# klkuhlm/unconfined

Measured on AMD Instinct MI355X. Metric: (t,r) drawdown points/sec, Neuman-1974 1024x256 sweep; max |rel err| vs CPU ref, higher is better.
Workload: dtype f64

## Files before the change

unconfined_amd/csrc/ucf_device.h:

```cpp

#include "ucf_math.h"
#include "ucf_plan.h"
#include <cstdlib>

namespace UCF_NS {

using namespace ucfm;

#define UCF_STR_(x) #x
#define UCF_STR(x) UCF_STR_(x)
#define UCF_PI 3.14159265358979323846
#define UCF_EPS 2.220446049250313e-16

UCF_DEV double shfl_down1(double v) { return __shfl_down(v, 1, 64); }
UCF_DEV double shift_down1(double x)
{
    const int lo = __double2loint(x), hi = __double2hiint(x);
    const int l2 = __builtin_amdgcn_update_dpp(lo, lo, 0x130, 0xf, 0xf, false);
    const int h2 = __builtin_amdgcn_update_dpp(hi, hi, 0x130, 0xf, 0xf, false);
    return __hiloint2double(h2, l2);
}
UCF_DEV cplx shfl_down1(cplx v) { return cmake(shift_down1(v.re), shift_down1(v.im)); }
UCF_DEV cplx bcast0(cplx v) { return cmake(__shfl(v.re, 0, 64), __shfl(v.im, 0, 64)); }
UCF_DEV double wave_max(double v)
{
#pragma unroll
    for (int off = 32; off >= 1; off >>= 1) v = fmax(v, __shfl_xor(v, off, 64));
    return v;
}
UCF_DEV void stat_add(long long* ctr, bool pred)
{
    if (ctr == nullptr) return;
    unsigned long long bal = __ballot(pred);
    if (bal != 0ull && (threadIdx.x & 63) == 0) atomicAdd((unsigned long long*)ctr, (unsigned long long)__popcll(bal));
}

#ifndef UCF_TU
#define UCF_TU -1
#endif
#define UCF_TU_HAS(L) (UCF_TU < 0 || UCF_TU == (L))

typedef double2 lds_c;
UCF_DEV cplx lds_ld(const lds_c* base, int slot, int lane) { lds_c v = base[slot * UCF_WAVE + lane]; return cmake(v.x, v.y); }
UCF_DEV void lds_st(lds_c* base, int slot, int lane, cplx z) { base[slot * UCF_WAVE + lane] = make_double2(z.re, z.im); }
#define UCF_PART 16
template <int PART = UCF_PART>
UCF_DEV cplx scr_ld(const lds_c* base, int slot, int lane) { lds_c v = base[slot * PART + (lane & (PART - 1))]; return cmake(v.x, v.y); }
template <int PART = UCF_PART>
UCF_DEV void scr_st(lds_c* base, int slot, int lane, cplx z) { base[slot * PART + (lane & (PART - 1))] = make_double2(z.re, z.im); }

#if UCF_FAST
UCF_DEV cplx cinv_plain_(cplx z)
{
    const double r = fast_rcp(z.re * z.re + z.im * z.im);
    return cmake(z.re * r, -(z.im * r));
}
#endif

UCF_DEV cplx lap_time(const ucf_dev_params& P, cplx p)
{
    if (P.timeType < 0) {
        const bool linear = P.timeType <= -101;
        const int n = linear ? -P.timeType - 100 : -P.timeType;
        cplx sum = cmake(0.0, 0.0);
        for (int k = 0; k < n; k++) {
            const cplx term = rscale(P.sched[n + k], cexp_(rscale(-P.sched[k], p)));
            sum = (k == 0) ? term : cadd(sum, term);
        }
        const cplx num = csub(sum, rscale(P.sched[2 * n + 1], cexp_(rscale(-P.sched[2 * n], p))));
        return cdiv(num, linear ? cmul(p, p) : p);
    }
    const double t1 = P.timePar[0], t2 = P.timePar[1];
    switch (P.timeType) {
    case 1: return cdiv(cexp_(cscale(p, -t1)), p);
    case 2: return csub(cdiv(cexp_(cscale(p, -t1)), p), cdiv(cexp_(cscale(p, -t2)), p));
    case 3: return cexp_(cscale(p, -t1));
    case 4: {
        cplx a = rdiv(1.0, csub(p, cmul(p, cexp_(cscale(p, -t1)))));
        cplx b = rsub(1.0, cexp_(cscale(p, -t2)));
        return cdiv(cmul(a, b), p);
    }
    case 5: return cdiv(cexp_(cscale(p, -t2)), cadd(p, cmul(p, cexp_(cscale(p, -t1)))));
    case 6: return cdiv(cmul(cexp_(cscale(p, -t2)), p), caddr(cmul(p, p), t1 * t1));
    case 7: return cmake(0.0, 0.0);
    case 8: {
        cplx ex = cexp_(cdivr(cscale(p, -t1), 2.0));
        cplx num = cmul(cexp_(cscale(p, -t2)), rsub(1.0, ex));
        return cdiv(num, cmul(radd(1.0, ex), p));
    }
    default: return cmake(__builtin_nan(""), __builtin_nan(""));
    }
}

struct k01 { cplx k0, k1; int ierr; };
UCF_DEV cplx clog_(cplx z) { return cmake(log(hypot(z.re, z.im)), atan2(z.im, z.re)); }

__device__ __noinline__ static k01 cbesk01_(cplx z)
{
    k01 out;
    out.k0 = cmake(0.0, 0.0); out.k1 = out.k0; out.ierr = 0;
    const double tol = UCF_EPS;
    const double elim = 2.303 * (1021.0 * log10(2.0) - 3.0);
    const double alim = elim + fmax(-(log10(2.0) * 52.0 * 2.303), -41.45);
    const double at1 = 0.78539816339744830962;
    const double pi = 4.0 * at1, hpi = 2.0 * at1, spi = 3.0 / (2.0 * at1);
    const double rthpi = sqrt(8.0 * at1) / 2.0, fpi = 1.89769999331517738, tth = 6.66666666666666666e-01;
    const double gamma_e = 5.77215664901532861e-01;
    const double xx = z.re, yy = z.im;
    if (xx == 0.0 && yy == 0.0) { out.ierr = 1; return out; }
    const double caz = hypot(xx, yy);
    if (caz > 1073741823.5) { out.ierr = 4; return out; }
    if (caz < UCF_DBL_MIN * 1.0e3) { out.ierr = 2; return out; }
    if (!(caz > tol) && -log(0.5 * caz) > elim) { out.ierr = 2; return out; }
    const cplx rz = cdiv(cmake(2.0, 0.0), z);
    cplx s1, s2;
    if (caz <= 2.0) {
        const cplx smu = clog_(rz);
        cplx f = cadd(rscale(-gamma_e, cmake(1.0, 0.0)), cscale(smu, 1.0));
        cplx p = cmake(0.5, 0.0), q = cmake(0.5, 0.0);
        s1 = f; s2 = p;
        double ak = 1.0, a1 = 1.0, bk = 1.0;
        cplx ck = cmake(1.0, 0.0);
        if (caz >= tol) {
            const cplx cz = cscale(cmul(z, z), 0.25);
            const double t1 = 0.25 * caz * caz;
            do {
                f = cdivr(cadd(cadd(cscale(f, ak), p), q), bk);
                p = cdivr(p, ak);
                q = cdivr(q, ak);
                const double rk = 1.0 / ak;
                ck = cscale(cmul(ck, cz), rk);
                s1 = cadd(s1, cmul(ck, f));
                s2 = cadd(s2, cmul(ck, csub(p, cscale(f, ak))));
                a1 = a1 * t1 * rk;
                bk = bk + ak + ak + 1.0;
                ak = ak + 1.0;
            } while (a1 > tol);
        }
        out.k0 = s1;
        out.k1 = cmul(s2, rz);
        return out;
    }
    if (xx > alim) { out.ierr = 2; return out; }
    cplx coef = cdiv(cmake(rthpi, 0.0), csqrt_(z));
    {
        double sn, cs;
        sincos_(yy, &sn, &cs);
        coef = cmul(coef, rscale(exp(-xx), cmake(cs, -sn)));
    }
    double ak = fabs(cos(pi * 0.0));
    double fhs = 0.25;
    double t1 = 52.0 * log10(2.0) * 3.321928094;
    t1 = fmin(fmax(t1, 12.0), 60.0);
    const double t2 = tth * t1 - 6.0;
    t1 = (xx == 0.0) ? hpi : fabs(atan(yy / xx));
    double fk;
// ... 1065 lines not shown
            }
        };
        for (; n < nabs; n++) {
            const double2 aa = row[n];
            sample_common S;
            S.clean3 = resume;
            sample_prepare<FAMILY>(P, aa.x, p, need_lay1, S, fdbuf, lane, lane_aux);
            for (int z = 0; z < nz; z++) {
                const cplx f = sample_z<FAMILY>(P, S, z);
                accumulate(n, aa.y, z, f);
            }
        }
        finish_item<LAYOUT, UCF_PART>(P, accTS, scr, areas_lds ? accGL : nullptr, areas, arg, W, pt, tD, tee, p, st, nt, ir0, totlap,
                                      hout, dhout);
    }
}

#if UCF_FAST
template <int FAMILY, bool MULTI>
__global__ void __launch_bounds__(256)
laptime_kernel(const ucf_dev_params P0, int nrows, const double* __restrict__ tDv, double2* __restrict__ ltab,
               const ucf_dev_params* __restrict__ Pv, int ppp, int pbase)
{
    const long long gid = (long long)blockIdx.x * blockDim.x + threadIdx.x;
    if (gid >= (long long)nrows * P0.np) return;
    const int m = (int)(gid / nrows), row = (int)(gid % nrows);
    const ucf_dev_params& P = item_params<MULTI>(P0, Pv, row + pbase, ppp);
    const double tee = 2.0 * tDv[row];
    const double sigma = P.alpha - P.logtol / (2.0 * tee);
    const cplx p = cmake(sigma, UCF_PI * m / tee);
    cplx lt = cscale(lap_time(P, p), fast_scale<FAMILY>(P));
    if (FAMILY == 5) lt = cmul(lt, cdiv(hstorage_A0(P, p), caddr(cscale(p, P.hs_tDb), 1.0)));
    ltab[gid] = make_double2(lt.re, lt.im);
}

#ifndef UCF_FOLD_WAVES
#define UCF_FOLD_WAVES 5
#endif
#ifndef UCF_UNFOLD_WAVES
#define UCF_UNFOLD_WAVES 4
#endif
#ifndef UCF_TAIL_LSPLIT_DEFAULT
#define UCF_TAIL_LSPLIT_DEFAULT 3
#endif
#ifndef UCF_KV
#define UCF_KV(FAMILY, FOLD) ((FAMILY) == 4 ? 0 : 4)
#endif
template <int FAMILY, int LAYOUT, int WAVES, bool MULTI, bool FOLD, bool LAY3, int NZC = 0, bool LAY1 = true, bool NOFOLD = false>
__global__ void __launch_bounds__(UCF_WAVE * UCF_IWPB, WAVES)
integrate_kernel(const ucf_dev_params P0, int npts, int per_point, int nr, int nsv, int svmin,
                 const double* __restrict__ tDv, const double* __restrict__ rDv, const int* __restrict__ svv,
                 const double2* __restrict__ tab, int nt, int ir0, double2* __restrict__ state, int* __restrict__ ndone,
                 int* __restrict__ todo, const ucf_dev_params* __restrict__ Pv, int ppp, int pbase, int lsplit,
                 const double2* __restrict__ ltab, int nrows, int nheadw, int nworkw, int* __restrict__ wcount)
{
    extern __shared__ lds_c lds[];
#ifdef UCF_K1_ASSUME
    const ucf_dev_params& P = P0;
    UCF_K1_ASSUME
#endif
    const int lane = threadIdx.x & (UCF_WAVE - 1), wv = __builtin_amdgcn_readfirstlane(threadIdx.x / UCF_WAVE);
    constexpr int EF = (FAMILY == 5) ? 1 : FAMILY;
    constexpr bool ZPAIR = FOLD && EF == 2 && NZC == 1;
    const int nz = NZC ? NZC : P0.nz, R = P0.R, nacc = P0.nacc, N = P0.N, ngl = P0.ngl;
    __builtin_assume(nz >= 1 && R >= 1 && nacc >= 1 && ngl >= 1);
    const int nabs = N + nacc * ngl;
    {
        const double2* __restrict__ gt = (const double2*)P0.sc_tab;
        for (int k = threadIdx.x; k < UCF_SC_ENTRIES; k += UCF_WAVE * UCF_IWPB) lds[k] = gt[k];
    }
    __syncthreads();
    const lds_c* sct = lds;
    const int lslots = (NZC ? R : R + 1) * nz;
    lds_c* const wlds = lds + UCF_SC_ENTRIES + (size_t)wv * lslots * UCF_WAVE;
    lds_c* accTS = wlds;
    lds_c* accCur = wlds + (size_t)R * nz * UCF_WAVE;
    int ustat = blockIdx.x * UCF_IWPB + wv - gridDim.x * UCF_IWPB;
    auto next_unit = [&]() {
        if (!wcount) return ustat += gridDim.x * UCF_IWPB;
        int u = 0;
        if (lane == 0) u = __hip_atomic_fetch_add(wcount, 1, __ATOMIC_RELAXED, __HIP_MEMORY_SCOPE_AGENT);
        return __builtin_amdgcn_readfirstlane(u);
    };
    for (int wi = next_unit(); wi < nworkw; wi = next_unit()) {
        const bool tail = wi >= nheadw;
        const int ls = tail ? (lsplit >> 8) : (lsplit & 255), nsplit = 1 << ls;
        const int wj = tail ? wi - nheadw : wi;
        const int pt = (tail ? (nheadw >> (lsplit & 255)) : 0) + (wj >> ls), sub = wj & (nsplit - 1);
        auto part_bound = [&](int k) {
            if (k <= 0) return 0;
            if (k >= nsplit) return nabs;
            int j = (k * nabs / nsplit - N + ngl / 2) / ngl;
            j = j < 0 ? 0 : (j > nacc ? nacc : j);
            return N + j * ngl;
        };
        const int n0 = part_bound(sub), n1 = part_bound(sub + 1);
        if (n1 <= n0 && sub != 0) continue;
#ifdef UCF_TIMELINE
        const unsigned long long tl_t0 = __builtin_amdgcn_s_memtime();
#endif
        const work_item W = decode_item<LAYOUT>(P0, pt, lane, per_point, nr, nt, ir0, npts);
        const ucf_dev_params& P = item_params<MULTI>(P0, Pv, (LAYOUT == 3 ? W.plan * ppp : W.pidx) + pbase, ppp);
        bool need_lay1 = false, need_lay3 = false, need_lay12 = false;
        for (int z = 0; z < nz; z++) { need_lay1 |= (P.zLay[z] == 1); need_lay3 |= (P.zLay[z] == 3); need_lay12 |= (P.zLay[z] != 3); }
        const double tD = tDv[W.it], rD = rDv[W.ir];
        const int sv = (LAYOUT == 1) ? svmin : svv[W.it];
        const double2* __restrict__ row = tab + (size_t)(per_point ? W.pidx : (W.ir * nsv + (sv - svmin))) * nabs;
        const double tee = 2.0 * tD;
        const double sigma = P.alpha - P.logtol / (2.0 * tee);
        const cplx p = cmake(sigma, UCF_PI * W.mlap / tee);
        const double2 ltv = ltab[(size_t)(W.mlap < P0.np ? W.mlap : P0.np - 1) * nrows + W.it];
        const cplx lt = cmake(ltv.x, ltv.y);
        const lane_consts LC = make_lane_consts(P, p, lt);
        auto lt_again = [&]() {
            int it = W.it;
            asm volatile("" : "+v"(it));
            const double2 v = ltab[(size_t)(W.mlap < P0.np ? W.mlap : P0.np - 1) * nrows + it];
            return cmake(v.x, v.y);
        };
        double2* __restrict__ sti = state + (size_t)pt * state_slots(P0) * UCF_WAVE;
        double2* __restrict__ areas = sti + (size_t)(R + 1) * nz * UCF_WAVE;
        for (int s = 0; s < lslots; s++) lds_st(wlds, s, lane, cmake(0.0, 0.0));
        fast_common F;
        sc_ctx_init(F.sc, sct, UCF_KV(FAMILY, FOLD));
        const bool lane_ok = FAMILY != 2 || (fabs(LC.xifac.re) + fabs(LC.xifac.im) < 1.0e90);
        const int nlim = (__builtin_amdgcn_ballot_w64(!lane_ok) == 0) ? n1 : n0;

        int n = n0;
        double2 aa = row[n0 < nabs ? n0 : 0];
        int m = 0, jj = n0 > N ? (n0 - N) / ngl : 0;
        cplx acc0 = cmake(0.0, 0.0), acc1 = cmake(0.0, 0.0);
        int zph = 0;
        if constexpr (ZPAIR) {
            int stopped = 0;
            zph = 0;
            if (!MULTI && nlim > n0)
                zph = zpair_part_phase(P, LC, P.j0z[sv - 1 + (nlim > N ? (nlim - N + ngl - 1) / ngl : 0)] / rD);
            const int nts = nlim < N ? nlim : N;
            for (; n < nts; n++) {
                const double2 nxt = row[n + 1 < nabs ? n + 1 : n];
                F.sc.salt = n;
                if (!fast_eta_wave_zpair<!MULTI>(P, LC, aa.x, F, zph, 1)) { stopped = 1; break; }
                const cplx val = rscale(aa.y, fast_sample_zpair<!MULTI>(P, LC, F, zph, 1));
                const int n1 = n + 1;
                int tz = __builtin_ctz(n1);
                if (tz > R - 1) tz = R - 1;
                for (int sh = 0; sh <= tz; sh++) {
                    const int j = R - sh;
                    const double wl = P.ts_w[(size_t)(j - 1) * N + ((n1 >> sh) - 1)];
                    lds_st(accTS, j - 1, lane, cadd(lds_ld(accTS, j - 1, lane), rscale(wl, val)));
                }
                aa = nxt;
            }
            if (!stopped) for (; n < nlim; n++) {
                const double2 nxt = row[n + 1 < nabs ? n + 1 : n];
                F.sc.salt = n;
                const int last = m == ngl - 1;
                if (!fast_eta_wave_zpair<!MULTI>(P, LC, aa.x, F, zph, last)) break;
                const cplx fz = fast_sample_zpair<!MULTI>(P, LC, F, zph, last);
                acc0 = cmake(__builtin_fma(fz.re, aa.y, acc0.re), __builtin_fma(fz.im, aa.y, acc0.im));
                if (++m == ngl) {
                    const double lob = P.j0z[sv + jj - 1] / rD;
                    const double hib = P.j0z[sv + jj] / rD;
                    const double hw = (hib - lob) / 2.0;
                    const cplx ar = cmul(rscale(hw, acc0), lt_again());
                    areas[(size_t)jj * UCF_WAVE + lane] = make_double2(ar.re, ar.im);
                    acc0 = cmake(0.0, 0.0);
                    m = 0;
                    jj++;
                }
                aa = nxt;
            }
        } else
        for (; n < nlim; n++) {
            const double2 nxt = row[n + 1 < nabs ? n + 1 : n];
            const bool ts = n < N;
            F.sc.salt = n;
            if (!fast_eta_wave<EF, ZPAIR>(P, LC, aa.x, F)) break;
            if constexpr (!ZPAIR) fast_common_terms<EF, FOLD, LAY3, LAY1, NOFOLD, ZPAIR>(P, LC, aa.x, need_lay1, F, need_lay3, need_lay12);
            const int n1 = n + 1;
            int tz = __builtin_ctz(n1);
            if (tz > R - 1) tz = R - 1;
            for (int z = 0; z < nz; z++) {
                cplx fz;
                if constexpr (ZPAIR) fz = fast_sample_zpair<!MULTI>(P, LC, F, zph, 0);
                else fz = fast_sample_z<EF, FOLD, LAY3, LAY1, NOFOLD, ZPAIR>(P, F, z);
                if (ts) {
                    const cplx val = rscale(aa.y, fz);
                    for (int sh = 0; sh <= tz; sh++) {
                        const int j = R - sh;
                        const double wl = P.ts_w[(size_t)(j - 1) * N + ((n1 >> sh) - 1)];
                        const int slot = (j - 1) * nz + z;
                        lds_st(accTS, slot, lane, cadd(lds_ld(accTS, slot, lane), rscale(wl, val)));
                    }
                } else if (nz == 1 || (NZC == 2 && z == 0)) {
                    acc0 = cmake(__builtin_fma(fz.re, aa.y, acc0.re), __builtin_fma(fz.im, aa.y, acc0.im));
                } else if (NZC == 2) {
                    acc1 = cmake(__builtin_fma(fz.re, aa.y, acc1.re), __builtin_fma(fz.im, aa.y, acc1.im));
                } else {
                    const cplx a1 = lds_ld(accCur, z, lane);
                    lds_st(accCur, z, lane, cmake(__builtin_fma(fz.re, aa.y, a1.re), __builtin_fma(fz.im, aa.y, a1.im)));
                }
            }
            if (!ts && ++m == ngl) {
                const double lob = P.j0z[sv + jj - 1] / rD;
                const double hib = P.j0z[sv + jj] / rD;
                const double hw = (hib - lob) / 2.0;
                for (int z = 0; z < nz; z++) {
                    const cplx run = (nz == 1 || (NZC == 2 && z == 0)) ? acc0 : (NZC == 2 ? acc1 : lds_ld(accCur, z, lane));
                    const cplx ar = cmul(rscale(hw, run), lt);
                    areas[(size_t)(jj * nz + z) * UCF_WAVE + lane] = make_double2(ar.re, ar.im);
                    if (nz != 1 && NZC != 2) lds_st(accCur, z, lane, cmake(0.0, 0.0));
                }
                acc0 = acc1 = cmake(0.0, 0.0);
                m = 0;
                jj++;
            }
            aa = nxt;
        }
        if (sub == 0) {
            const cplx lte = ZPAIR ? lt_again() : lt;
            for (int s = 0; s < R * nz; s++) {
                const cplx v = cmul(lds_ld(wlds, s, lane), lte);
                sti[(size_t)s * UCF_WAVE + lane] = make_double2(v.re, v.im);
            }
            for (int s = R * nz; s < (R + 1) * nz; s++) sti[(size_t)s * UCF_WAVE + lane] = make_double2(0.0, 0.0);
        }
#ifdef UCF_TIMELINE
        if (sub == 0) {
            const unsigned long long tl_t1 = __builtin_amdgcn_s_memtime();
            const unsigned hwid = __builtin_amdgcn_s_getreg(63492);
            if (lane == 0) sti[(size_t)(R * nz) * UCF_WAVE + 0] = make_double2(__longlong_as_double((long long)tl_t0), __longlong_as_double((long long)tl_t1));
            if (lane == 1) sti[(size_t)(R * nz) * UCF_WAVE + 1] = make_double2((double)hwid, (double)__builtin_amdgcn_s_getreg(63508));
        }
#endif
        if (n < n1 && lane == 0) {
            const int nrep = (n < N) ? n : n - m;
            if (atomicMin(&ndone[pt], nrep) == nabs) todo[1 + atomicAdd(&todo[0], 1)] = pt;
        }
    }
}

#endif

template <int FAMILY, int LAYOUT>
__global__ void __launch_bounds__(UCF_WAVE, 3)
integrate_generic_kernel(const ucf_dev_params P, int npts, int per_point, int nr, int nsv, int svmin,
                         const double* __restrict__ tDv, const double* __restrict__ rDv, const int* __restrict__ svv,
                         const double2* __restrict__ tab, int nt, int ir0, double2* __restrict__ state, int* __restrict__ ndone)
{
    extern __shared__ lds_c lds[];
    const int lane = threadIdx.x;
    const int nz = P.nz, R = P.R, nacc = P.nacc, N = P.N, ngl = P.ngl;
    const int nabs = N + nacc * ngl;
    lds_c* accTS = lds;
    lds_c* accCur = lds + (size_t)R * nz * UCF_WAVE;
    lds_c* fdbuf = accCur + (size_t)nz * UCF_WAVE;
    bool need_lay1 = false;
    for (int z = 0; z < nz; z++) need_lay1 |= (P.zLay[z] == 1);
    for (int pt = blockIdx.x; pt < npts; pt += gridDim.x) {
        const work_item W = decode_item<LAYOUT>(P, pt, lane, per_point, nr, nt, ir0, npts);
        const double tD = tDv[W.it], rD = rDv[W.ir];
        const int sv = (LAYOUT == 1) ? svmin : svv[W.it];
        const double2* __restrict__ row = tab + (size_t)(per_point ? W.pidx : (W.ir * nsv + (sv - svmin))) * nabs;
        const double tee = 2.0 * tD;
        const double sigma = P.alpha - P.logtol / (2.0 * tee);
        const cplx p = cmake(sigma, UCF_PI * W.mlap / tee);
        const cplx lt = lap_time(P, p);
        const cplx lane_aux = (FAMILY == 5) ? hstorage_A0(P, p) : cmake(0.0, 0.0);
        double2* __restrict__ sti = state + (size_t)pt * state_slots(P) * UCF_WAVE;
        double2* __restrict__ areas = sti + (size_t)(R + 1) * nz * UCF_WAVE;
        for (int s = 0; s < (R + 1) * nz; s++) lds_st(lds, s, lane, cmake(0.0, 0.0));
        int m = 0, jj = 0;
        for (int n = 0; n < nabs; n++) {
            const double2 aa = row[n];
            sample_common S;
            S.clean3 = false;
            sample_prepare<FAMILY>(P, aa.x, p, need_lay1, S, fdbuf, lane, lane_aux);
            const bool ts = n < N;
            for (int z = 0; z < nz; z++) {
                const cplx val = cmul(rscale(aa.y, sample_z<FAMILY>(P, S, z)), lt);
                if (ts) {
                    const int n1 = n + 1;
                    for (int j = 1; j <= R; j++) {
                        const int sh = R - j;
                        if ((n1 & ((1 << sh) - 1)) == 0) {
                            const double w = P.ts_w[(size_t)(j - 1) * N + ((n1 >> sh) - 1)];
                            const int slot = (j - 1) * nz + z;
                            lds_st(accTS, slot, lane, cadd(lds_ld(accTS, slot, lane), rscale(w, val)));
                        }
                    }
                } else {
                    cplx acc = cadd(lds_ld(accCur, z, lane), cscale(val, P.tab_premul ? 1.0 : P.gl_w[m]));
                    if (m == ngl - 1) {
                        const double lob = P.j0z[sv + jj - 1] / rD;
                        const double hib = P.j0z[sv + jj] / rD;
                        acc = rscale((hib - lob) / 2.0, acc);
                        areas[(size_t)(jj * nz + z) * UCF_WAVE + lane] = make_double2(acc.re, acc.im);
                        acc = cmake(0.0, 0.0);
                    }
                    lds_st(accCur, z, lane, acc);
                }
            }
            if (!ts && ++m == ngl) { m = 0; jj++; }
        }
        for (int s = 0; s < (R + 1) * nz; s++) sti[(size_t)s * UCF_WAVE + lane] = lds[s * UCF_WAVE + lane];
        if (lane == 0) ndone[pt] = nabs;
    }
}

template <int LAYOUT, int PART, bool WREG, int MODE = 0>
__global__ void __launch_bounds__(UCF_WAVE, (LAYOUT == 0 || (WREG && MODE != 1)) ? 3 : 4)
finish_kernel(const ucf_dev_params P, int npts, int per_point, int nr, int nsv, int svmin,
              const double* __restrict__ tDv, const double* __restrict__ rDv, const int* __restrict__ svv,
              double* __restrict__ hout, double* __restrict__ dhout, ucf_stats* st, int nt, int ir0,
              double2* __restrict__ totlap, const double2* __restrict__ state, const int* __restrict__ ndone, int* __restrict__ defer)
{
    extern __shared__ lds_c lds[];
    const int lane = threadIdx.x;
    const int nz = P.nz, R = P.R, nacc = P.nacc;
    const int nabs = P.N + nacc * P.ngl;
    lds_c* accTS = lds;
    lds_c* scr = lds + (size_t)R * nz * UCF_WAVE;
    const int nloop = (MODE == 2) ? defer[0] : npts;
    for (int wi = blockIdx.x; wi < nloop; wi += gridDim.x) {
// ... 831 lines not shown
```

unconfined_amd/csrc/ucf_fastpath.h:

```cpp
#pragma once

namespace UCF_NS {

#define UCF_UNIFORM_BLOCK() asm volatile("" ::: "memory")
#define UCF_UNIFORM_BLOCK_F(FAMILY) do { if constexpr ((FAMILY) != 4) UCF_UNIFORM_BLOCK(); } while (0)

struct fprim {
    double ch, sh, ei, sn, cs;
};

template <bool POS, bool SMALLY = false>
UCF_DEV fprim prim_from_e(double x, double ax, double e, double ei, double y, const sc_ctx& sc)
{
    const int salt = sc.salt;
    fprim f;
    f.ei = ei;
    const double he = 0.5 * e;
    f.ch = __builtin_fma(0.5, ei, he);
    double s;
    if (ax < 0.35) {
        const double x2 = ax * ax;
        double pl = addk(mulk(x2, UCF_KHERE(1.0 / 6227020800.0, salt)), UCF_KHERE(1.0 / 39916800.0, salt));
        pl = fmak(pl, x2, UCF_KHERE(1.0 / 362880.0, salt));
        pl = fmak(pl, x2, UCF_KHERE(1.0 / 5040.0, salt));
// ... 46 lines not shown
    f.sh = 0.5 * (e - ei);
    f.sn = __builtin_fma(a.sn, b.cs, -(a.cs * b.sn));
    f.cs = __builtin_fma(a.cs, b.cs, a.sn * b.sn);
    return f;
}
UCF_DEV cplx pcosh(const fprim& f) { return cmake(f.ch * f.cs, f.sh * f.sn); }
UCF_DEV cplx psinh(const fprim& f) { return cmake(f.sh * f.cs, f.ch * f.sn); }
UCF_DEV cplx pexpneg(const fprim& f) { return cmake(f.ei * f.cs, -(f.ei * f.sn)); }

UCF_DEV cplx expneg_direct(double x, double y, const sc_ctx& sc)
{
    const double ei = exp_tab_(-x, sc);
    double sn, cs;
    sincos_tab_(y, sc, &sn, &cs);
    return cmake(ei * cs, -(ei * sn));
}

UCF_DEV cplx expneg_small(double x, double y, const sc_ctx& sc)
{
    const double ei = exp_tab_(-x, sc);
    double sn, cs;
    sincos_small_(y, sc, &sn, &cs);
    return cmake(ei * cs, -(ei * sn));
}
UCF_DEV void prim_pair_small(double x, double y, double zD, double xcap, const sc_ctx& sc, fprim* f, fprim* fz)
{
    double xc;
    asm("v_min_f64 %0, %1, %2" : "=v"(xc) : "v"(x), "s"(xcap));
    const double xz = xc * zD;
    const double e = exp_tab_(xc, sc), ez = exp_tab_(xz, sc);
    const double r = fast_rcp(e * ez);
    *f = prim_from_e<true, true>(xc, xc, e, r * ez, y, sc);
    *fz = prim_from_e<true, true>(xz, xz, ez, r * e, y * zD, sc);
}

UCF_DEV cplx cfma(cplx a, cplx b, cplx c)
{
    return cmake(__builtin_fma(a.re, b.re, __builtin_fma(-a.im, b.im, c.re)), __builtin_fma(a.re, b.im, __builtin_fma(a.im, b.re, c.im)));
}
UCF_DEV cplx cfnma(cplx a, cplx b, cplx c)
{
    return cmake(__builtin_fma(-a.re, b.re, __builtin_fma(a.im, b.im, c.re)), __builtin_fma(-a.re, b.im, __builtin_fma(-a.im, b.re, c.im)));
}
UCF_DEV cplx cinv_plain(cplx z)
{
    const double r = fast_rcp(z.re * z.re + z.im * z.im);
    return cmake(z.re * r, -(z.im * r));
}
UCF_DEV cplx cinv_scaled(cplx z)
{
    const double m = fmax(fabs(z.re), fabs(z.im));
    const int il = __builtin_amdgcn_frexp_exp(m) - 1;
    const double c = ldexp(z.re, -il), d = ldexp(z.im, -il);
    const double r = fast_rcp(c * c + d * d);
    return cmake(ldexp(c * r, -il), ldexp(-(d * r), -il));
}

UCF_DEV cplx cinv_auto(cplx z)
{
    const double m = fmax(fabs(z.re), fabs(z.im));
    if (__builtin_amdgcn_ballot_w64(!(m < 1.0e150 && m > 1.0e-150)) == 0) return cinv_plain(z);
    return cinv_scaled(z);
}

struct lane_consts {
    cplx p, lt, xifac;
    cplx fdB1;
    cplx mnpv;
};

UCF_DEV lane_consts make_lane_consts(const ucf_dev_params& P, cplx p, cplx lt)
{
    lane_consts L;
    L.p = p;
    L.lt = lt;
    cplx xf = rscale(P.alphaD, cinv_plain(p));
    if (P.model == 3) {
        cplx sum = cmake(0.0, 0.0);
        for (int j = 0; j < P.MoenchM; j++) sum = cadd(sum, cinv_plain(radd(1.0, cscale(p, P.MoenchInvGamma[j]))));
        xf = cmul(cscale(xf, (double)P.MoenchM), cinv_plain(sum));
    }
    L.xifac = xf;
    L.fdB1 = cscale(cscale(cscale(p, P.fd_beta0), P.fd_expmb2), P.inv_kappa);
    L.mnpv = radd(1.0, cscale(p, P.mn_vartheta * P.mn_c3));
    return L;
}

struct fast_common {
    sc_ctx sc;
    cplx th, eta, ff1, ff2, inv_she, she, che, top, g3, inv_den, ex1;
    cplx chz0;
    fprim p1;
    int have_p1;
    cplx mn_uod;
#ifdef UCF_SINGLE_RCP
    cplx q, den;
#endif
    cplx fd_s1;
    cplx top3, fd_s13;
    bool small_eta, fd_use, fd_use3;
    int any_small, any_large;
};

template <int FAMILY>
UCF_DEV double fast_scale(const ucf_dev_params& P)
{
    if (FAMILY == 0 || FAMILY == 3) return 2.0;
    if (FAMILY == 5) return P.inv_bD;
    return (FAMILY == 2 && P.model == 4) ? 2.0 : 2.0 * P.inv_bD;
}

template <int FAMILY, bool PAIR = false>
UCF_DEV bool fast_eta(const ucf_dev_params& P, const lane_consts& L, double a, fast_common& S)
{
    const double a2 = a * a;
    const cplx q = caddr(L.p, a2);
#ifdef UCF_SINGLE_RCP
    S.q = q;
#endif
    double mq = 0.0;
    if (PAIR && FAMILY != 0) {
        double r;
        rsq_pair(q.re * q.re + q.im * q.im, &mq, &r);
        S.th = cmake(q.re * r, -(q.im * r));
    } else {
        const double r = fast_rcp(q.re * q.re + q.im * q.im);
        S.th = cmake(q.re * r, -(q.im * r));
    }
    if (FAMILY == 0) return q.re > 0.0;
    {
        const double qr = q.re * P.inv_kappa, qi = q.im * P.inv_kappa;
        double r, hr;
        const double d = PAIR ? mq * P.inv_kappa : sqrt_only(__builtin_fma(qr, qr, qi * qi));
        sqrt_hrsqrt(0.5 * (d + qr), &r, &hr);
        S.eta = cmake(r, qi * hr);
    }
    return (S.eta.re <= P.fast_eta_max) & (q.re > 0.0) & (fabs(S.eta.im) < P.fast_im_max);
}
template <int FAMILY, bool PAIR = false>
UCF_DEV bool fast_eta_wave(const ucf_dev_params& P, const lane_consts& L, double a, fast_common& S)
{
    (void)fast_eta<FAMILY, PAIR>(P, L, a, S);
    const cplx q = caddr(L.p, a * a);
    unsigned long long bad = __builtin_amdgcn_ballot_w64(!(q.re > 0.0));
    if (FAMILY != 0) {
        bad |= __builtin_amdgcn_ballot_w64(!(S.eta.re <= P.fast_eta_max));
        bad |= __builtin_amdgcn_ballot_w64(!(fabs(S.eta.im) < P.fast_im_max));
    }
    return bad == 0;
}

#ifndef UCF_ZPAIR_PHASES
#define UCF_ZPAIR_PHASES 3
#endif
enum {
    UCF_PH_RANGE = 1,
    UCF_PH_IM = 2,
    UCF_PH_LARGE = 4,
    UCF_PH_YS = 8,
    UCF_PH_YL = 16
};
UCF_DEV int zpair_part_phase(const ucf_dev_params& P, const lane_consts& L, double a_max)
{
    if (!(UCF_ZPAIR_PHASES & 2)) return 0;
    const double lim = 0.99 * P.fast_eta_max;
    const bool ok = (L.p.re > 0.0) & (lim > 0.0) & ((__builtin_fma(a_max, a_max, fabs(L.p.re) + fabs(L.p.im)) * P.inv_kappa) < lim * lim);
    return __builtin_amdgcn_ballot_w64(!ok) == 0 ? UCF_PH_RANGE : 0;
}
template <bool UNI>
UCF_DEV bool fast_eta_wave_zpair(const ucf_dev_params& P, const lane_consts& L, double a, fast_common& S, int& ph, int may_set)
{
    if constexpr (!UNI) return fast_eta_wave<2, true>(P, L, a, S);
    (void)fast_eta<2, true>(P, L, a, S);
    unsigned long long bad = 0;
    if (!(ph & UCF_PH_RANGE)) {
        const cplx q = caddr(L.p, a * a);
        bad |= __builtin_amdgcn_ballot_w64(!(q.re > 0.0));
        bad |= __builtin_amdgcn_ballot_w64(!(S.eta.re <= P.fast_eta_max));
        UCF_UNIFORM_BLOCK();
    }
    if (!(ph & UCF_PH_IM)) {
        const double ai = fabs(S.eta.im);
        bad |= __builtin_amdgcn_ballot_w64(!(ai < P.fast_im_max));
        if ((UCF_ZPAIR_PHASES & 2) && may_set && __builtin_amdgcn_ballot_w64(!(ai < 0.5 * P.fast_im_max)) == 0) ph |= UCF_PH_IM;
        UCF_UNIFORM_BLOCK();
    }
    return bad == 0;
}

template <int FAMILY, bool FOLD = false, bool LAY3 = true, bool LAY1 = true, bool NOFOLD = false, bool ZPAIR = false>
UCF_DEV void fast_common_terms(const ucf_dev_params& P, const lane_consts& L, double a, bool need_lay1_in, fast_common& S,
                               bool need_lay3_in = false, bool need_lay12 = true)
{
    static_assert(!ZPAIR || (FOLD && FAMILY == 2), "ZPAIR: folded water-table kernels only");
    const double a2 = a * a;
    if (FAMILY == 0) return;
    if (FAMILY == 3) {
        const fprim p1 = prim<true>(S.eta.re, S.eta.im, S.sc);
        S.che = pcosh(p1);
        S.she = psinh(p1);
        const double wr = __builtin_fma(a2, P.mn_c3, L.mnpv.re), wi = L.mnpv.im;
        double vr, hr;
        sqrt_hrsqrt(0.5 * (sqrt_only(__builtin_fma(wr, wr, wi * wi)) + wr), &vr, &hr);
        const cplx u = cmake(P.mn_u0 * (1.0 - vr), -(P.mn_u0 * (wi * hr)));
        const cplx Delta0 = cfnma(u, S.che, cmul(S.eta, S.she));
        S.mn_uod = cmul(u, cinv_auto(Delta0));
        return;
    }
    const bool hantush = NOFOLD || !(FAMILY == 2 && P.model == 4);
    const bool z1 = FOLD || (!NOFOLD && P.fold_dD != 0), z2 = FOLD || (!NOFOLD && P.fold_lD1 != 0);
    const bool need_lay1 = (FOLD || !LAY1) ? false : need_lay1_in;
    const bool need_lay3 = (FOLD || !LAY3) ? false : need_lay3_in;
    S.small_eta = (FAMILY != 2) || (S.eta.re < P.maxexp);
    S.any_small = ((FAMILY != 2) || (__builtin_amdgcn_ballot_w64(S.small_eta) != 0)) ? 1 : 0;
    S.any_large = ((FAMILY == 2) && (__builtin_amdgcn_ballot_w64(!S.small_eta) != 0)) ? 1 : 0;
    const bool need_p1 = (hantush && (!(z1 && z2) || need_lay1)) || FAMILY == 4 || (FAMILY == 2 && S.any_small);
    S.have_p1 = (need_p1 && !z2) ? 1 : 0;
    fprim p1;
    if (ZPAIR && need_p1) {
        fprim pz;
        prim_pair(S.eta.re, S.eta.im, P.zD[0], P.maxexp, S.sc, &p1, &pz);
        S.chz0 = pcosh(pz);
        S.che = pcosh(p1);
        S.she = psinh(p1);
        S.ex1 = cmake(0.0, 0.0);
    } else if (need_p1) {
        p1 = prim<true>(S.eta.re, S.eta.im, S.sc);
        if (!z2) S.p1 = p1;
        S.che = pcosh(p1);
        S.she = psinh(p1);
        if (need_lay1) S.ex1 = pexpneg(p1);
        else S.ex1 = cmake(0.0, 0.0);
    } else {
        S.che = S.she = S.ex1 = cmake(0.0, 0.0);
    }
    if (hantush) {
        fprim pd;
        if (!z1) { pd = prim<true>(S.eta.re * P.dD, S.eta.im * P.dD, S.sc); S.ff1 = psinh(pd); }
        else S.ff1 = cmake(0.0, 0.0);
        fprim pl;
        if (!z2) { pl = prim<true>(S.eta.re * P.lD1, S.eta.im * P.lD1, S.sc); S.ff2 = psinh(pl); }
        else S.ff2 = cmake(0.0, 0.0);
        if (!(z1 && z2) || need_lay1) S.inv_she = cinv_auto(S.she);
        if (need_lay1) {
            const cplx exl = z2 ? cmake(1.0, 0.0) : pexpneg(pl);
            S.g3 = csub(exl, cmul(cadd(S.ff1, cmul(S.ex1, S.ff2)), S.inv_she));
        }
        if (FAMILY != 1) {
            S.top = S.top3 = S.th;
            if (!(z1 && z2)) {
                if (need_lay12) {
                    cplx g1;
                    if (z1) g1 = cmake(1.0, 0.0);
                    else if (P.share_g1top == 1) g1 = pcosh(pd);
                    else if (P.share_g1top == 2) g1 = csub(pcosh(pd), cmul(rscale(P.g1_delta, S.eta), S.ff1));
                    else { const double c = P.dD1 - 1.0; g1 = pcosh(prim(S.eta.re * c, S.eta.im * c, S.sc)); }
                    const cplx udp = csub(g1, cmul(cadd(cmul(S.ff1, S.che), S.ff2), S.inv_she));
                    S.top = cmul(udp, S.th);
                }
                if (need_lay3) {
                    cplx sd1 = S.she;
                    if (!z1) {
                        const double x1 = S.eta.re * P.dD1;
                        if (__builtin_amdgcn_ballot_w64(!(x1 >= 1.0)) == 0) sd1 = psinh(prim_difference(p1, pd));
                        else sd1 = psinh(prim(x1, S.eta.im * P.dD1, S.sc));
                    }
                    const cplx udp = cmul(z2 ? sd1 : csub(sd1, S.ff2), S.inv_she);
                    S.top3 = cmul(udp, S.th);
                }
            }
        }
    } else {
        S.top = S.top3 = S.th;
    }
    if (FAMILY == 2) {
        const cplx xi = cmul(S.eta, L.xifac);
        if (P.beta != 0.0) {
            const cplx one_bex = radd(1.0, cmul(rscale(P.beta, S.eta), xi));
            if (S.small_eta) S.inv_den = cinv_plain(cfma(one_bex, S.che, cmul(xi, S.she)));
            else S.inv_den = cinv_plain(cadd(one_bex, xi));
        } else {
            if (S.small_eta) S.inv_den = cinv_plain(cfma(xi, S.she, S.che));
            else S.inv_den = cinv_plain(radd(1.0, xi));
        }
#ifdef UCF_SINGLE_RCP
        if (FOLD || !hantush) {
            cplx den;
            if (P.beta != 0.0) {
                const cplx one_bex = radd(1.0, cmul(rscale(P.beta, S.eta), xi));
                den = S.small_eta ? cfma(one_bex, S.che, cmul(xi, S.she)) : cadd(one_bex, xi);
            } else {
                den = S.small_eta ? cfma(xi, S.she, S.che) : radd(1.0, xi);
            }
            S.den = den;
            S.inv_den = cinv_auto(cmul(S.q, den));
        }
#endif
    }
    if (FAMILY == 4) {
        const int n = P.order;
        const double h = P.fd_h, invhsq = P.fd_invhsq, b3h = P.fd_beta3 / h;
        const double B2 = a2 * P.inv_kappa;
        const double csup = invhsq - b3h, K = csup * invhsq, bmid = b3h - 2.0 * invhsq - B2;
        const cplx B1 = L.fdB1;
        const cplx cc = cmake((b3h - invhsq - B2) - B1.re * P.fd_e[0], -(B1.im * P.fd_e[0]));
        const cplx eoh = cscale(S.eta, 1.0 / h);
        const cplx b1 = csub(cmul(cc, S.che), cmul(eoh, S.she));
        (void)n;
        const cplx iB2 = fd_inverse_B2(P, B1, bmid, invhsq, b3h, K);
        const cplx a2v = cscale(S.che, invhsq);
        const cplx B1p = csub(b1, cmul(rscale(csup, a2v), iB2));
        const cplx iB1p = cinv_scaled(B1p);
        const cplx v1 = cneg(cmul(cc, S.top)), v2 = rscale(-invhsq, S.top);
        const cplx v1p = csub(v1, cmul(rscale(csup, iB2), v2));
        S.fd_s1 = cmul(v1p, iB1p);
        S.fd_use = (fabs(S.fd_s1.re) + fabs(S.fd_s1.im)) > 2.3e-308;
        S.fd_s13 = S.fd_s1;
        S.fd_use3 = S.fd_use;
        if (need_lay3) {
            const cplx w1 = cneg(cmul(cc, S.top3)), w2 = rscale(-invhsq, S.top3);
            S.fd_s13 = cmul(csub(w1, cmul(rscale(csup, iB2), w2)), iB1p);
            S.fd_use3 = (fabs(S.fd_s13.re) + fabs(S.fd_s13.im)) > 2.3e-308;
        }
    }
}

template <int FAMILY>
UCF_DEV bool fast_prepare(const ucf_dev_params& P, const lane_consts& L, double a, bool need_lay1, fast_common& S)
{
    if (!fast_eta<FAMILY>(P, L, a, S)) return false;
    bool need_lay3 = false, need_lay12 = false;
    for (int z = 0; z < P.nz; z++) { need_lay3 |= (P.zLay[z] == 3); need_lay12 |= (P.zLay[z] != 3); }
    fast_common_terms<FAMILY>(P, L, a, need_lay1, S, need_lay3, need_lay12);
    return true;
}

template <int FAMILY, bool FOLD = false, bool LAY3 = true, bool LAY1 = true, bool NOFOLD = false, bool ZPAIR = false>
UCF_DEV cplx fast_hantush_z(const ucf_dev_params& P, const fast_common& S, double zD, int lay_in, cplx* chz_out,
                            cplx* exz_out)
{
    const bool z1 = FOLD || (!NOFOLD && P.fold_dD != 0), z2 = FOLD || (!NOFOLD && P.fold_lD1 != 0);
    const int lay = (FOLD || (!LAY1 && lay_in == 1)) ? 2 : lay_in;
    const bool need_chz = (lay == 1) || !z1 || (FAMILY == 2 && S.any_small) || FAMILY == 4;
    cplx chz = cmake(1.0, 0.0);
    fprim pz;
    if (ZPAIR) { if (need_chz) chz = S.chz0; }
    else if (need_chz) { pz = prim<true>(S.eta.re * zD, S.eta.im * zD, S.sc); chz = pcosh(pz); }
    *chz_out = chz;
    cplx udp;
    if (lay == 1) {
        udp = cmul(S.g3, chz);
    } else {
        cplx g2 = cmake(0.0, 0.0);
        const bool need_1z = !z2;
        fprim p1z;
        if (z2 && FAMILY == 2 && S.any_large) {
            const double c = 1.0 - zD;
            *exz_out = expneg_direct(S.eta.re * c, S.eta.im * c, S.sc);
            UCF_UNIFORM_BLOCK_F(FAMILY);
        }
        if (need_1z) {
            if (need_chz && S.have_p1 && zD >= 0.0 && zD <= 1.0) p1z = prim_difference(S.p1, pz);
            else
            { const double c = 1.0 - zD; p1z = prim(S.eta.re * c, S.eta.im * c, S.sc); }
        }
        if (!z2 && FAMILY == 2 && S.any_large) { *exz_out = pexpneg(p1z); UCF_UNIFORM_BLOCK_F(FAMILY); }
        cplx f2c = cmake(0.0, 0.0);
        if (!z2) f2c = cmul(S.ff2, pcosh(p1z));
        if (lay == 2 || !LAY3) {
            if (z1 && z2) { UCF_UNIFORM_BLOCK_F(FAMILY); return S.th; }
            cplx num = f2c;
            if (!z1) { num = cadd(cmul(S.ff1, chz), f2c); UCF_UNIFORM_BLOCK_F(FAMILY); }
            g2 = cmul(num, S.inv_she);
            udp = rsub(1.0, g2);
            UCF_UNIFORM_BLOCK_F(FAMILY);
        } else {
            const double ca = 2.0 - zD - P.dD, cb = zD - P.dD;
            const cplx sa = psinh(prim(S.eta.re * ca, S.eta.im * ca, S.sc));
            const cplx sb = psinh(prim(S.eta.re * cb, S.eta.im * cb, S.sc));
            const cplx num = cmake(__builtin_fma(0.5, sa.re + sb.re, -f2c.re), __builtin_fma(0.5, sa.im + sb.im, -f2c.im));
            udp = cmul(num, S.inv_she);
        }
    }
    const cplx res = cmul(udp, S.th);
    UCF_UNIFORM_BLOCK_F(FAMILY);
    return res;
}

template <int FAMILY, bool FOLD = false, bool LAY3 = true, bool LAY1 = true, bool NOFOLD = false, bool ZPAIR = false>
UCF_DEV cplx fast_sample_z(const ucf_dev_params& P, const fast_common& S, int iz)
{
    const double zD = P.zD[iz];
    const int lay = P.zLay[iz];
    cplx chz, exz = cmake(0.0, 0.0);
    if (FAMILY == 0) return S.th;
    if (FAMILY == 3) {
        const cplx cz = pcosh(prim<true>(S.eta.re * zD, S.eta.im * zD, S.sc));
        return cfma(S.th, cmul(S.mn_uod, cz), S.th);
    }
    if (FAMILY == 1) return fast_hantush_z<1, FOLD, LAY3, LAY1, NOFOLD>(P, S, zD, lay, &chz, &exz);
    if (FAMILY == 4) {
        const cplx sH = fast_hantush_z<4, FOLD, LAY3, LAY1, NOFOLD>(P, S, zD, lay, &chz, &exz);
        if (!FOLD && LAY3 && lay == 3) return S.fd_use3 ? cadd(sH, cmul(S.fd_s13, chz)) : sH;
        return S.fd_use ? cadd(sH, cmul(S.fd_s1, chz)) : sH;
    }
    cplx u;
    if (!NOFOLD && P.model == 4) {
        u = S.th;
        if (S.any_small) chz = ZPAIR ? S.chz0 : pcosh(prim(S.eta.re * zD, S.eta.im * zD, S.sc));
        if (S.any_large) { const double c = 1.0 - zD; exz = expneg_direct(S.eta.re * c, S.eta.im * c, S.sc); }
    } else {
        u = fast_hantush_z<2, FOLD, LAY3, LAY1, NOFOLD, ZPAIR>(P, S, zD, lay, &chz, &exz);
        if (LAY1 && S.any_large && lay == 1) { const double c = 1.0 - zD; exz = expneg_direct(S.eta.re * c, S.eta.im * c, S.sc); }
    }
#ifdef UCF_SINGLE_RCP
    if (FOLD || (!NOFOLD && P.model == 4)) return cmul(csub(S.den, S.small_eta ? chz : exz), S.inv_den);
#endif
    const cplx top = (!FOLD && LAY3 && (NOFOLD || P.model != 4) && lay == 3) ? S.top3 : S.top;
    cplx g = chz;
    if (S.any_large) {
        g = S.small_eta ? chz : exz;
        asm volatile("" ::: "memory");
    }
    return cfnma(cmul(top, g), S.inv_den, u);
}

template <bool UNI, bool SMALLY>
UCF_DEV void zpair_arm_small(const ucf_dev_params& P, const lane_consts& L, const fast_common& S, double zD, cplx* g, cplx* den)
{
    fprim p1, pz;
    if (SMALLY) prim_pair_small(S.eta.re, S.eta.im, zD, P.maxexp, S.sc, &p1, &pz);
    else prim_pair_min<UNI>(S.eta.re, S.eta.im, zD, P.maxexp, S.sc, &p1, &pz);
    *g = pcosh(pz);
    const cplx che = pcosh(p1), she = psinh(p1);
    const cplx xi = cmul(S.eta, L.xifac);
    if (P.beta != 0.0) *den = cfma(radd(1.0, cmul(rscale(P.beta, S.eta), xi)), che, cmul(xi, she));
    else *den = cfma(xi, she, che);
}
template <bool SMALLY>
UCF_DEV void zpair_arm_large(const ucf_dev_params& P, const lane_consts& L, const fast_common& S, double x, double y, cplx* g, cplx* den)
{
    *g = SMALLY ? expneg_small(x, y, S.sc) : expneg_direct(x, y, S.sc);
    const cplx xi = cmul(S.eta, L.xifac);
    if (P.beta != 0.0) *den = cadd(radd(1.0, cmul(rscale(P.beta, S.eta), xi)), xi);
    else *den = radd(1.0, xi);
}
template <bool UNI>
UCF_DEV cplx fast_sample_zpair(const ucf_dev_params& P, const lane_consts& L, const fast_common& S, int& ph, int may_set)
{
    constexpr bool SHORT = UNI && (UCF_ZPAIR_PHASES & 1);
    const double zD = P.zD[0];
    int form = 2;
    if (!UNI || !(ph & UCF_PH_LARGE)) {
        const bool small_eta = S.eta.re < P.maxexp;
        const bool any_small = __builtin_amdgcn_ballot_w64(small_eta) != 0, any_large = __builtin_amdgcn_ballot_w64(!small_eta) != 0;
        form = !any_large ? 0 : (any_small ? 1 : 2);
        if (UNI && (UCF_ZPAIR_PHASES & 2) && may_set && form == 2 && __builtin_amdgcn_ballot_w64(!(S.eta.re > P.maxexp * (1.0 + 0x1p-20))) == 0) ph |= UCF_PH_LARGE;
        UCF_UNIFORM_BLOCK();
    }
    cplx den, g;
    if (form == 0) {
        if (SHORT && may_set && !(ph & UCF_PH_YS)) {
            if (__builtin_amdgcn_ballot_w64(!(fabs(S.eta.im) < UCF_SC_SMALL)) == 0) ph |= UCF_PH_YS | UCF_PH_YL;
            UCF_UNIFORM_BLOCK();
        }
        if (SHORT && (ph & UCF_PH_YS)) {
            zpair_arm_small<UNI, true>(P, L, S, zD, &g, &den);
            UCF_UNIFORM_BLOCK();
        } else {
            zpair_arm_small<UNI, false>(P, L, S, zD, &g, &den);
            UCF_UNIFORM_BLOCK();
        }
    } else if (form == 2) {
        const double c = 1.0 - zD;
        const double x = S.eta.re * c, y = S.eta.im * c;
        if (SHORT && may_set && !(ph & UCF_PH_YL)) {
            if (__builtin_amdgcn_ballot_w64(!(fabs(y) < UCF_SC_SMALL)) == 0) ph |= UCF_PH_YL;
            UCF_UNIFORM_BLOCK();
        }
        if (SHORT && (ph & UCF_PH_YL)) {
            zpair_arm_large<true>(P, L, S, x, y, &g, &den);
            UCF_UNIFORM_BLOCK();
        } else {
            zpair_arm_large<false>(P, L, S, x, y, &g, &den);
            UCF_UNIFORM_BLOCK();
        }
    } else {
        const bool small_eta = S.eta.re < P.maxexp;
        fprim p1, pz;
        prim_pair_min<UNI>(S.eta.re, S.eta.im, zD, P.maxexp, S.sc, &p1, &pz);
        const cplx chz = pcosh(pz), che = pcosh(p1), she = psinh(p1);
        const cplx xi = cmul(S.eta, L.xifac);
        if (P.beta != 0.0) {
            const cplx one_bex = radd(1.0, cmul(rscale(P.beta, S.eta), xi));
            den = small_eta ? cfma(one_bex, che, cmul(xi, she)) : cadd(one_bex, xi);
        } else {
            den = small_eta ? cfma(xi, she, che) : radd(1.0, xi);
        }
        const double c = 1.0 - zD;
        const cplx exz = expneg_direct(S.eta.re * c, S.eta.im * c, S.sc);
        g = small_eta ? chz : exz;
        UCF_UNIFORM_BLOCK();
    }
    const double r = fast_rcp(__builtin_fma(den.im, den.im, den.re * den.re));
    const cplx inv_den = cmake(den.re * r, -(den.im * r));
    return cfnma(cmul(S.th, g), inv_den, S.th);
}


}
```

Before: 9.022 million.

## Classify zpair Bessel-zero intervals upfront and run branch-free specialized sample loops

```diff
diff --git a/unconfined_amd/csrc/ucf_device.h b/unconfined_amd/csrc/ucf_device.h
--- a/unconfined_amd/csrc/ucf_device.h
+++ b/unconfined_amd/csrc/ucf_device.h
@@ -2,6 +2,7 @@
 #include "ucf_math.h"
 #include "ucf_plan.h"
 #include <cstdlib>
+#include <type_traits>
 
 namespace UCF_NS {
 
@@ -1373,6 +1374,57 @@
                 }
                 aa = nxt;
             }
+#if UCF_ZPAIR_INTERVALS
+            auto proven_interval = [&](auto cls, auto beta) {
+                for (int i = 0; i < ngl; i++, n++) {
+                    const double2 nxt = row[n + 1 < nabs ? n + 1 : n];
+                    F.sc.salt = n;
+                    (void)fast_eta<2, true>(P, LC, aa.x, F);
+                    const cplx fz = fast_sample_zpair_proven<decltype(cls)::value, decltype(beta)::value>(P, LC, F);
+                    acc0 = cmake(__builtin_fma(fz.re, aa.y, acc0.re), __builtin_fma(fz.im, aa.y, acc0.im));
+                    aa = nxt;
+                }
+            };
+            auto proven_class = [&](auto cls) {
+                if (P.beta != 0.0) proven_interval(cls, std::true_type());
+                else proven_interval(cls, std::false_type());
+            };
+            if (!stopped) while (n < nlim) {
+                const double lob = P.j0z[sv + jj - 1] / rD;
+                const double hib = P.j0z[sv + jj] / rD;
+                int cls = UCF_IV_UNPROVEN;
+                if constexpr (!MULTI) {
+                    int known;
+                    cls = zpair_interval_class(P, LC, lob, hib, P.zD[0], &known);
+                    zph |= known;
+                }
+                if (cls == UCF_IV_CS_TAB) proven_class(std::integral_constant<int, UCF_IV_CS_TAB>());
+                else if (cls == UCF_IV_CS_SHORT) proven_class(std::integral_constant<int, UCF_IV_CS_SHORT>());
+                else if (cls == UCF_IV_EX_TAB) proven_class(std::integral_constant<int, UCF_IV_EX_TAB>());
+                else if (cls == UCF_IV_EX_SHORT) proven_class(std::integral_constant<int, UCF_IV_EX_SHORT>());
+                else {
+                    for (m = 0; m < ngl; m++, n++) {
+                        const double2 nxt = row[n + 1 < nabs ? n + 1 : n];
+                        F.sc.salt = n;
+                        const int last = m == ngl - 1;
+                        if (!fast_eta_wave_zpair<!MULTI>(P, LC, aa.x, F, zph, last)) { stopped = 1; break; }
+                        const cplx fz = fast_sample_zpair<!MULTI>(P, LC, F, zph, last);
+                        acc0 = cmake(__builtin_fma(fz.re, aa.y, acc0.re), __builtin_fma(fz.im, aa.y, acc0.im));
+                        aa = nxt;
+                    }
+                    if (stopped) break;
+                }
+                UCF_UNIFORM_BLOCK();
+                {
+                    const double hw = (hib - lob) / 2.0;
+                    const cplx ar = cmul(rscale(hw, acc0), lt_again());
+                    areas[(size_t)jj * UCF_WAVE + lane] = make_double2(ar.re, ar.im);
+                    acc0 = cmake(0.0, 0.0);
+                    m = 0;
+                    jj++;
+                }
+            }
+#else
             if (!stopped) for (; n < nlim; n++) {
                 const double2 nxt = row[n + 1 < nabs ? n + 1 : n];
                 F.sc.salt = n;
@@ -1392,6 +1444,7 @@
                 }
                 aa = nxt;
             }
+#endif
         } else
         for (; n < nlim; n++) {
             const double2 nxt = row[n + 1 < nabs ? n + 1 : n];
diff --git a/unconfined_amd/csrc/ucf_fastpath.h b/unconfined_amd/csrc/ucf_fastpath.h
--- a/unconfined_amd/csrc/ucf_fastpath.h
+++ b/unconfined_amd/csrc/ucf_fastpath.h
@@ -222,6 +222,9 @@
 
 #ifndef UCF_ZPAIR_PHASES
 #define UCF_ZPAIR_PHASES 3
+#endif
+#ifndef UCF_ZPAIR_INTERVALS
+#define UCF_ZPAIR_INTERVALS 1
 #endif
 enum {
     UCF_PH_RANGE = 1,
@@ -495,7 +498,7 @@
     return cfnma(cmul(top, g), S.inv_den, u);
 }
 
-template <bool UNI, bool SMALLY>
+template <bool UNI, bool SMALLY, int KB = -1>
 UCF_DEV void zpair_arm_small(const ucf_dev_params& P, const lane_consts& L, const fast_common& S, double zD, cplx* g, cplx* den)
 {
     fprim p1, pz;
@@ -504,15 +507,15 @@
     *g = pcosh(pz);
     const cplx che = pcosh(p1), she = psinh(p1);
     const cplx xi = cmul(S.eta, L.xifac);
-    if (P.beta != 0.0) *den = cfma(radd(1.0, cmul(rscale(P.beta, S.eta), xi)), che, cmul(xi, she));
+    if (KB < 0 ? P.beta != 0.0 : KB != 0) *den = cfma(radd(1.0, cmul(rscale(P.beta, S.eta), xi)), che, cmul(xi, she));
     else *den = cfma(xi, she, che);
 }
-template <bool SMALLY>
+template <bool SMALLY, int KB = -1>
 UCF_DEV void zpair_arm_large(const ucf_dev_params& P, const lane_consts& L, const fast_common& S, double x, double y, cplx* g, cplx* den)
 {
     *g = SMALLY ? expneg_small(x, y, S.sc) : expneg_direct(x, y, S.sc);
     const cplx xi = cmul(S.eta, L.xifac);
-    if (P.beta != 0.0) *den = cadd(radd(1.0, cmul(rscale(P.beta, S.eta), xi)), xi);
+    if (KB < 0 ? P.beta != 0.0 : KB != 0) *den = cadd(radd(1.0, cmul(rscale(P.beta, S.eta), xi)), xi);
     else *den = radd(1.0, xi);
 }
 template <bool UNI>
@@ -525,7 +528,9 @@
         const bool small_eta = S.eta.re < P.maxexp;
         const bool any_small = __builtin_amdgcn_ballot_w64(small_eta) != 0, any_large = __builtin_amdgcn_ballot_w64(!small_eta) != 0;
         form = !any_large ? 0 : (any_small ? 1 : 2);
-        if (UNI && (UCF_ZPAIR_PHASES & 2) && may_set && form == 2 && __builtin_amdgcn_ballot_w64(!(S.eta.re > P.maxexp * (1.0 + 0x1p-20))) == 0) ph |= UCF_PH_LARGE;
+        double mx = P.maxexp;
+        if (UCF_ZPAIR_INTERVALS) asm volatile("" : "+s"(mx));
+        if (UNI && (UCF_ZPAIR_PHASES & 2) && may_set && form == 2 && __builtin_amdgcn_ballot_w64(!(S.eta.re > mx * (1.0 + 0x1p-20))) == 0) ph |= UCF_PH_LARGE;
         UCF_UNIFORM_BLOCK();
     }
     cplx den, g;
@@ -577,5 +582,51 @@
     return cfnma(cmul(S.th, g), inv_den, S.th);
 }
 
-
-}
+enum {
+    UCF_IV_UNPROVEN = 0,
+    UCF_IV_CS_TAB = 1,
+    UCF_IV_CS_SHORT = 2,
+    UCF_IV_EX_TAB = 3,
+    UCF_IV_EX_SHORT = 4
+};
+UCF_DEV int zpair_interval_class(const ucf_dev_params& P, const lane_consts& L, double lob, double hib, double zD, int* ph_proven)
+{
+    *ph_proven = 0;
+    fast_common T;
+    (void)fast_eta<2, true>(P, L, hib, T);
+    const double re_hi = T.eta.re;
+    (void)fast_eta<2, true>(P, L, lob, T);
+    const double re_lo = T.eta.re, im_lo = fabs(T.eta.im);
+    const bool in_range = (L.p.re > 0.0) & (re_hi * 1.01 <= P.fast_eta_max) & (im_lo * 2.0 < P.fast_im_max);
+    if (__builtin_amdgcn_ballot_w64(!in_range) != 0) return UCF_IV_UNPROVEN;
+    *ph_proven = UCF_PH_IM;
+    const bool ys = __builtin_amdgcn_ballot_w64(!(im_lo < UCF_SC_SMALL)) == 0;
+    const bool yl = ys || __builtin_amdgcn_ballot_w64(!(im_lo * (1.0 - zD) < UCF_SC_SMALL)) == 0;
+    if (ys) *ph_proven |= UCF_PH_YS;
+    if (yl) *ph_proven |= UCF_PH_YL;
+    if (__builtin_amdgcn_ballot_w64(!(re_hi * (1.0 + 0x1p-20) < P.maxexp)) == 0) return ys ? UCF_IV_CS_SHORT : UCF_IV_CS_TAB;
+    if (__builtin_amdgcn_ballot_w64(!(re_lo * (1.0 - 0x1p-20) > P.maxexp)) == 0) {
+        *ph_proven |= UCF_PH_LARGE;
+        return yl ? UCF_IV_EX_SHORT : UCF_IV_EX_TAB;
+    }
+    return UCF_IV_UNPROVEN;
+}
+template <int CLS, bool BETA>
+UCF_DEV cplx fast_sample_zpair_proven(const ucf_dev_params& P, const lane_consts& L, const fast_common& S)
+{
+    const double zD = P.zD[0];
+    cplx den, g;
+    if (CLS == UCF_IV_CS_TAB || CLS == UCF_IV_CS_SHORT) {
+        zpair_arm_small<true, CLS == UCF_IV_CS_SHORT, BETA ? 1 : 0>(P, L, S, zD, &g, &den);
+    } else {
+        const double c = 1.0 - zD;
+        const double x = S.eta.re * c, y = S.eta.im * c;
+        zpair_arm_large<CLS == UCF_IV_EX_SHORT, BETA ? 1 : 0>(P, L, S, x, y, &g, &den);
+    }
+    const double r = fast_rcp(__builtin_fma(den.im, den.im, den.re * den.re));
+    const cplx inv_den = cmake(den.re * r, -(den.im * r));
+    return cfnma(cmul(S.th, g), inv_den, S.th);
+}
+
+
+}
```

Result: faster. 9.275 million (median of 6 runs) (+2.8%).
